# una-auxme/MeshGraphNets.jl

Measured on AMD Instinct MI355X. Metric: processor-step edges/s, higher is better.
Workload: dtype f32; 1 GPU; M-1M jittered-grid triangulation 1000x1000: N=1000000 nodes, E=5992002 directed edges, L=128, hidden_layers=2, 15 processor steps per bench step, fp32 storage, fp16x2 split MFMA (every fp32 operand = two fp16 pieces after a power-of-two scaling per weight chunk / per activation row, three exact piece products per fp32 product on v_mfma_f32_32x32x16_f16), fp32 accumulate; held to the fp32 tolerance; partition=single partition, edge_order=engine re-sorts by receiver once per trajectory (mgn_set_graph)

## Files before the change

### meshgraphnets.jl_amd/csrc/frag.hpp

```cpp
#pragma once
#include <hip/hip_runtime.h>
#include <stdint.h>

#include "kernels.h"

namespace mgn {

typedef float f32x16 __attribute__((ext_vector_type(16)));
typedef float f32x4 __attribute__((ext_vector_type(4)));
typedef float f32x2 __attribute__((ext_vector_type(2)));

#define DEVINL __device__ __forceinline__
#define PHASE_FENCE() __builtin_amdgcn_sched_barrier(0)
#define MGN_PRIO 1
#define OPAQUE_LANE()                          \
    int lane = lane0;                          \
    asm volatile("" : "+v"(lane));             \
    const int c = lane & 31, h = lane >> 5
constexpr float LN_EPS = 1e-5f;
constexpr int NUM_XCD = 8;

constexpr int STRIDE_ROW = 2, STRIDE_TILE = 64;

DEVINL const f32x4* row_ptr(const float* base, int64_t row, int L, int h) {
// ... 262 lines not shown
    const float rstd = ln_rstd(q * invL, gamma, 32 * NT);
    const f32x4* g4 = reinterpret_cast<const f32x4*>(gamma) + h;
    const f32x4* b4 = reinterpret_cast<const f32x4*>(beta) + h;
#pragma unroll
    for (int t = 0; t < NT; ++t)
#pragma unroll
        for (int g = 0; g < 4; ++g) {
            const f32x4 gv = g4[2 * (4 * t + g)];
            const f32x4 bv = b4[2 * (4 * t + g)];
#pragma unroll
            for (int i = 0; i < 4; ++i) x[t][4 * g + i] = x[t][4 * g + i] * rstd * gv[i] + bv[i];
        }
}

DEVINL void copy_to_lds(float* dst, const float* __restrict__ src, int nfloats) {
    const f32x4* s4 = reinterpret_cast<const f32x4*>(src);
    f32x4* d4 = reinterpret_cast<f32x4*>(dst);
    for (int i = threadIdx.x; i < nfloats / 4; i += blockDim.x) d4[i] = s4[i];
}

DEVINL void copy_to_lds_vec(f32x4* d4, const f32x4* __restrict__ s4, int n4) {
    constexpr int B = 8;
    const int bd = blockDim.x;
    for (int i = threadIdx.x; i < n4; i += B * bd) {
        f32x4 v[B];
#pragma unroll
        for (int u = 0; u < B; ++u) {
            const int k = i + u * bd;
            v[u] = s4[k < n4 ? k : i];
        }
#pragma unroll
        for (int u = 0; u < B; ++u) {
            const int k = i + u * bd;
            if (k < n4) d4[k] = v[u];
        }
    }
}

DEVINL void copy_to_lds_sel(float* dst, const float* __restrict__ src, int nfloats, bool fast) {
    if (fast) copy_to_lds_vec(reinterpret_cast<f32x4*>(dst), reinterpret_cast<const f32x4*>(src), nfloats / 4);
    else copy_to_lds(dst, src, nfloats);
}

#define MGN_COOP_PF 4
constexpr int COOP_PF = MGN_COOP_PF;

struct CoopRing {
    f32x4 r[COOP_PF];
};
DEVINL void coop_prime(CoopRing& ring, const float* wt, int lane) {
    const f32x4* wv = reinterpret_cast<const f32x4*>(wt) + lane;
#pragma unroll
    for (int p = 0; p < COOP_PF; ++p) ring.r[p] = wv[p * 64];
}
template <bool FENCE>
DEVINL void coop_chain_primed(f32x16& acc, const f32x16 (&in)[4], const float* wt, int lane, CoopRing& ring) {
    const f32x4* wv = reinterpret_cast<const f32x4*>(wt) + lane;
#pragma unroll
    for (int m = 0; m < 16; ++m) {
        const f32x4 a = ring.r[m % COOP_PF];
        if (m + COOP_PF < 16) ring.r[m % COOP_PF] = wv[(m + COOP_PF) * 64];
        if constexpr (FENCE) __builtin_amdgcn_sched_barrier(0);
#pragma unroll
        for (int i = 0; i < 4; ++i)
            acc = __builtin_amdgcn_mfma_f32_32x32x2f32(a[i], in[m >> 2][4 * (m & 3) + i], acc, 0, 0, 0);
        if constexpr (FENCE) __builtin_amdgcn_sched_barrier(0);
    }
}
template <bool FENCE>
DEVINL void coop_chain(f32x16& acc, const f32x16 (&in)[4], const float* wt, int lane) {
    CoopRing ring;
    coop_prime(ring, wt, lane);
    if constexpr (FENCE) __builtin_amdgcn_sched_barrier(0);
    coop_chain_primed<FENCE>(acc, in, wt, lane, ring);
}

DEVINL void coop_exchange(f32x16 (&full)[4], const f32x16& mine, f32x4* xch, int wave, int lane) {
#pragma unroll
    for (int g = 0; g < 4; ++g) {
        f32x4 v;
        v[0] = mine[4 * g + 0]; v[1] = mine[4 * g + 1]; v[2] = mine[4 * g + 2]; v[3] = mine[4 * g + 3];
        xch[(4 * wave + g) * 64 + lane] = v;
    }
    __syncthreads();
#pragma unroll
    for (int m = 0; m < 16; ++m) {
        const f32x4 v = xch[m * 64 + lane];
        full[m >> 2][4 * (m & 3) + 0] = v[0]; full[m >> 2][4 * (m & 3) + 1] = v[1];
        full[m >> 2][4 * (m & 3) + 2] = v[2]; full[m >> 2][4 * (m & 3) + 3] = v[3];
    }
}

DEVINL void tab_quarter(f32x16& q, const float* tab, int t, int h) { load_quarter(q, reinterpret_cast<const f32x4*>(tab) + h, 2, t); }

DEVINL void relu_quarter(f32x16& q) {
#pragma unroll
    for (int k = 0; k < 16; ++k) q[k] = fmaxf(q[k], 0.f);
}

DEVINL void zero_quarter(f32x16& q) {
#pragma unroll
    for (int k = 0; k < 16; ++k) q[k] = 0.f;
}

DEVINL void coop_layer_norm(f32x16& mine, const f32x16 (&full)[4], const float* gamma, const float* beta, int t, int h) {
    float s = 0.f;
#pragma unroll
    for (int u = 0; u < 4; ++u)
#pragma unroll
        for (int k = 0; k < 16; ++k) s += full[u][k];
    s += __shfl_xor(s, 32, 64);
    const float mean = s * (1.0f / 128);
    float q = 0.f;
#pragma unroll
    for (int u = 0; u < 4; ++u)
#pragma unroll
        for (int k = 0; k < 16; ++k) {
            const float d = full[u][k] - mean;
            q += d * d;
        }
    q += __shfl_xor(q, 32, 64);
    const float rstd = ln_rstd(q * (1.0f / 128), gamma, 128);
    f32x16 gq, bq;
    tab_quarter(gq, gamma, t, h);
    tab_quarter(bq, beta, t, h);
#pragma unroll
    for (int k = 0; k < 16; ++k) mine[k] = (mine[k] - mean) * rstd * gq[k] + bq[k];
}

DEVINL void coop_layer_norm_reg(f32x16& mine, const f32x16 (&full)[4], const f32x16& gq, const f32x16& bq, const float* lnp) {
    float s = 0.f;
#pragma unroll
    for (int u = 0; u < 4; ++u)
#pragma unroll
        for (int k = 0; k < 16; ++k) s += full[u][k];
    s += __shfl_xor(s, 32, 64);
    const float mean = s * (1.0f / 128);
    float q = 0.f;
#pragma unroll
    for (int u = 0; u < 4; ++u)
#pragma unroll
        for (int k = 0; k < 16; ++k) {
            const float d = full[u][k] - mean;
            q += d * d;
        }
    q += __shfl_xor(q, 32, 64);
    const float rstd = ln_rstd_at(q * (1.0f / 128), lnp);
#pragma unroll
    for (int k = 0; k < 16; ++k) mine[k] = (mine[k] - mean) * rstd * gq[k] + bq[k];
}

#define MGN_SPREAD_ROUNDS 24
#define MGN_SPREAD_ROUNDS_NODE MGN_SPREAD_ROUNDS
struct TileWalk {
    int tile, end, stride;
    DEVINL TileWalk(int ntiles, int wave, int spread_rounds = MGN_SPREAD_ROUNDS) {
        const int wpb = blockDim.x >> 6;
        const int xcd = blockIdx.x % NUM_XCD;
        const int per = (ntiles + NUM_XCD - 1) / NUM_XCD;
        const int nb = (gridDim.x - xcd + NUM_XCD - 1) / NUM_XCD;
        end = min(xcd * per + per, ntiles);
        stride = nb * wpb;
        const bool spread = per < spread_rounds * stride;
        tile = xcd * per + (spread ? wave * nb + (int)(blockIdx.x / NUM_XCD) : (int)(blockIdx.x / NUM_XCD) * wpb + wave);
    }
};


}
```

### meshgraphnets.jl_amd/csrc/split.hip

```cpp

#include "kernels.h"
#include "tile_common.hpp"
#include "split_common.hpp"
#include "launch.hpp"

namespace mgn {


template <int D> struct SpRing { u32x4 r2[D], r3[D]; };
template <bool G2, bool G3, bool RELU, int D, bool G1 = false, int OFF = 0, bool PRIMED = false, bool NEXT = false>
DEVINL void sp_layer_otf(f32x16 (&acc)[4], const f32x16 (&in)[4], const u32x4* p1, const u32x4* p2, const u32x4* p3, int lane,
                         SpRing<D>* carry = nullptr, const u32x4* nx2 = nullptr, const u32x4* nx3 = nullptr) {
    const u32x4* w1 = p1 + lane;
    const u32x4* w2 = p2 + lane;
    const u32x4* w3 = p3 + lane;
    const N16Buf b1 = n16_buf(G1 ? p1 : nullptr), b2 = n16_buf(G2 ? p2 : nullptr), b3 = n16_buf(G3 ? p3 : nullptr);
    const unsigned voff = (unsigned)lane * 16u;
#define SP_G1(IDX) n16_ldu(b1, voff, (IDX) * 1024)
#define SP_G2(IDX) n16_ldu(b2, voff, (IDX) * 1024)
#define SP_G3(IDX) n16_ldu(b3, voff, (IDX) * 1024)
    static_assert(!(PRIMED || NEXT) || !G1, "ring carry-over is written for the mid / lo streams");
    u32x4 r1[G1 ? D : 1], r2[G2 ? D : 1], r3[G3 ? D : 1];
    if constexpr (PRIMED) {
#pragma unroll
// ... 369 lines not shown
        EST(3);
        const int reff = ix.r >= 0 ? r : (-4 - c);
        const int rprev = lane_prev(reff);
        const int rnext = lane_next(reff);
        const bool head = (c == 0) || (reff != rprev);
        const unsigned hm = (unsigned)__ballot(head);
        const int start = 31 - __clz((int)(hm & (0xFFFFFFFFu >> (31 - c))));
        const int st_in = max(start, c & 16);
        const bool c1 = (c - 1 >= st_in), c2 = (c - 2 >= st_in), c4 = (c - 4 >= st_in), c8 = (c - 8 >= st_in);
        const bool cx = (c >= 16) && (start <= 15);
        EST(4);
        PHASE_FENCE();
        asm volatile("s_nop 1");
        RG_SCAN_LEVEL(acc, c1, "row_shr:1 row_mask:0xf bank_mask:0xf");
        RG_SCAN_LEVEL(acc, c2, "row_shr:2 row_mask:0xf bank_mask:0xf");
        RG_SCAN_LEVEL(acc, c4, "row_shr:4 row_mask:0xf bank_mask:0xf");
        RG_SCAN_LEVEL(acc, c8, "row_shr:8 row_mask:0xf bank_mask:0xf");
        RG_SCAN_LEVEL(acc, cx, "row_bcast:15 row_mask:0xa bank_mask:0xf");
        PHASE_FENCE();
        EST(5);
        const bool tail = valid && ((c == 31) || (reff != rnext));
        const int r_first = __builtin_amdgcn_readfirstlane(reff);
        const bool sl = (start == 0) && (ix.r_before == r_first);
        const bool sr = (c == 31) && (ix.r_after == reff);
        const bool to_carry = sl || sr;
        f32x4* dst = to_carry ? prow_ptr(a.CARRY, (int64_t)2 * tile + (sl ? 0 : 1), L, h) : tile_ptr(a.AGG, r >> 5, L, 32 * h + (r & 31));
        if (tail) store_frag<NT>(dst, to_carry ? STRIDE_PROW : STRIDE_TILE, acc);
        EST(6);
        PHASE_FENCE();
        load_frag<NT>(acc, prow_ptr(a.Q, ixn.r >= 0 ? ixn.r : 0, L, h), STRIDE_PROW);
        EST(7);
        ix = ixn;
        tw.tile += tw.stride;
    }
}

#define MGN_RINGH_AHEAD 2
template <int W>
struct Rh {
    static constexpr int WPL = 32 / W;
    static constexpr int NW = 3 * WPL;
    static constexpr int NB = MGN_RINGH_AHEAD + 1;
    static constexpr int BUF = W * 64;
    static_assert(NW % NB == 0 && NW % 2 == 0, "static window -> buffer / slot mapping");
};
template <int LPT> struct RhPend { u32x4 v[2][LPT]; };
struct RhFrag {
    u32x4 h, l;
};
template <int W, int LYR>
DEVINL RhFrag rh_first(const u32x4* hi, const u32x4* ring, int lane) {
    constexpr int b = (Rh<W>::WPL * LYR) % Rh<W>::NB;
    RhFrag f;
    f.h = hi[lane];
    f.l = ring[b * Rh<W>::BUF];
    return f;
}
struct RhSrc {
    const u32x4* lo[3];
};
template <int W, int LYR, int FIN, int RFS = 0, int NWV = 8, bool WRAP = false>
DEVINL void h2_layer_ring(f32x16 (&acc)[4], f32x16 (&in)[4], const u32x4* hi, const u32x4* hi_next, u32x4* ring, const RhSrc& src,
                          RhFrag& nx, RhPend<W / NWV>& pend, int lane, int tid, float sx, float cfin = 0.f, const float* btab = nullptr,
                          const f32x4* rf = nullptr, const N16Buf* rfb = nullptr) {
    constexpr int ROT = 2;
    constexpr int WPL = Rh<W>::WPL, NW = Rh<W>::NW, BUF = Rh<W>::BUF, NB = Rh<W>::NB, AHEAD = MGN_RINGH_AHEAD;
    f32x4 side[2 * ROT];
    if constexpr (!WRAP && RFS > 0) {
#pragma unroll
        for (int m = 0; m < 2 * ROT; ++m) side[m] = rf[m * RFS];
    }
    auto bias = [&](int sn, int u) {
        f32x2 b = {0.f, 0.f};
        if constexpr (FIN == 2) b = *reinterpret_cast<const f32x2*>(btab + 8 * (4 * (sn >> 1) + 2 * (sn & 1) + (u >> 1)) + 2 * (u & 1));
        return b;
    };
    unsigned ph[4], pl[4];
#pragma unroll
    for (int u = 0; u < 4; ++u) {
        const f32x2 b = bias(0, u);
        h2_split_pair<FIN>(ph[u], pl[u], in[0][2 * u], in[0][2 * u + 1], sx, cfin, b[0], b[1]);
    }
    constexpr int LPT = W / NWV;
    unsigned voff = (unsigned)tid * 16u;
    asm volatile("" : "+v"(voff));
    __builtin_amdgcn_sched_barrier(0);
#pragma unroll
    for (int s = 0; s < 8; ++s) {
        unsigned nh[4], nl[4];
#pragma unroll
        for (int t = 0; t < 4; ++t) {
            const int it = 4 * s + t;
            const int gw = WPL * LYR + it / W;
            const u32x4 a1 = nx.h, a2 = nx.l;
            if (it % W == 0) {
                const int g2 = (gw + AHEAD) % NW, l2 = g2 / WPL, w2 = g2 % WPL;
#pragma unroll
                for (int i = 0; i < LPT; ++i)
                    pend.v[AHEAD == 2 ? 0 : gw % 2][i] = *reinterpret_cast<const u32x4*>(reinterpret_cast<const char*>(src.lo[l2] + w2 * W * 64 + i * NWV * 64) + voff);
            }
            if constexpr (RFS > 0) {
                if ((t & 1) && s < 8 - ROT) {
                    f32x4 v;
                    if constexpr (WRAP) v = n16_ld(*rfb, (unsigned)lane * 16u, (2 * s + (t >> 1)) * 1024);
                    else v = rf[(2 * (s + ROT) + (t >> 1)) * RFS];
#pragma unroll
                    for (int i = 0; i < 4; ++i) in[s >> 1][8 * (s & 1) + 4 * (t >> 1) + i] = v[i];
                }
            }
            if (it + 1 < 32) {
                const int gn = WPL * LYR + (it + 1) / W;
                nx.h = hi[(it + 1) * 64 + lane];
                nx.l = ring[(gn % NB) * BUF + ((it + 1) % W) * 64];
            } else if (LYR < 2) {
                nx = rh_first<W, (LYR + 1) % 3>(hi_next, ring, lane);
            }
            if (it % W == W - 2) {
                const int b2 = (gw + 2) % NB;
                const int slot = AHEAD == 2 ? 0 : (gw + 1) % 2;
#pragma unroll
                for (int i = 0; i < LPT; ++i) ring[b2 * BUF + i * NWV * 64 + tid - lane] = pend.v[slot][i];
            }
            if (s < 7) {
                const int sn = s + 1;
                const f32x2 b = bias(sn, t);
                h2_split_pair<FIN>(nh[t], nl[t], in[sn >> 1][8 * (sn & 1) + 2 * t], in[sn >> 1][8 * (sn & 1) + 2 * t + 1], sx, cfin, b[0], b[1]);
            }
            const sp_f16x8 bh = h2_op(ph), bl = h2_op(pl);
            acc[t] = __builtin_amdgcn_mfma_f32_32x32x16_f16(h2_wop(a2), bh, acc[t], 0, 0, 0);
            acc[t] = __builtin_amdgcn_mfma_f32_32x32x16_f16(h2_wop(a1), bl, acc[t], 0, 0, 0);
            acc[t] = __builtin_amdgcn_mfma_f32_32x32x16_f16(h2_wop(a1), bh, acc[t], 0, 0, 0);
            __builtin_amdgcn_sched_barrier(0);
            if (it % W == W - 1) ring_barrier();
        }
#pragma unroll
        for (int u = 0; u < 4; ++u) {
            ph[u] = nh[u];
            pl[u] = nl[u];
        }
    }
    if constexpr (RFS > 0 && !WRAP) {
        f32x16 r[4];
#pragma unroll
        for (int u = 0; u < 8; ++u)
#pragma unroll
            for (int j = 0; j < 8; ++j)
                r[u >> 1][8 * (u & 1) + j] = u < ROT ? side[2 * u + (j >> 2)][j & 3] : in[(u - ROT) >> 1][8 * ((u - ROT) & 1) + j];
#pragma unroll
        for (int t = 0; t < 4; ++t) in[t] = r[t];
    }
}

#define MGN_RINGH_PHASE_UNITS 6
#define MGN_RINGH_W 8
template <int NWV>
__global__ __launch_bounds__(NWV * 64, NWV / 4) void k_edge_ring_h(const EdgeArgs a) {
    constexpr int NT = 4, L = 128, PC = 16384;
    constexpr int W = MGN_RINGH_W;
    constexpr int BUF = Rh<W>::BUF;
    extern __shared__ __attribute__((aligned(16))) float smem[];
    uint16_t* wl = reinterpret_cast<uint16_t*>(smem);
    copy_to_lds16(wl, a.splith[2], PC, true);
    copy_to_lds16(wl + PC, a.splith[0], PC, true);
    copy_to_lds16(wl + 2 * PC, a.splith[1], PC, true);
    const int lane0 = threadIdx.x & 63;
    const int wave = __builtin_amdgcn_readfirstlane(threadIdx.x >> 6);
    const int tid = (int)threadIdx.x;
    u32x4* ringbase = reinterpret_cast<u32x4*>(wl + 3 * PC);
    float* tb = reinterpret_cast<float*>(ringbase + Rh<W>::NB * BUF);
    copy_to_lds(tb, a.tabs, T_COUNT * L);
    RhSrc src;
    RhPend<W / NWV> pend;
    {
        const u32x4* g[3] = {reinterpret_cast<const u32x4*>(a.splith[2]), reinterpret_cast<const u32x4*>(a.splith[0]),
                             reinterpret_cast<const u32x4*>(a.splith[1])};
#pragma unroll
        for (int l = 0; l < 3; ++l) src.lo[l] = g[l] + 2048;
#pragma unroll
        for (int w = 0; w < 2; ++w)
#pragma unroll
            for (int i = 0; i < W / NWV; ++i) ringbase[w * BUF + i * NWV * 64 + tid] = src.lo[0][w * W * 64 + i * NWV * 64 + tid];
#pragma unroll
        for (int i = 0; i < W / NWV; ++i) {
            pend.v[1][i] = src.lo[(2 * W) / 32][((2 * W) % 32) * 64 + i * NWV * 64 + tid];
            pend.v[0][i] = pend.v[1][i];
        }
    }
    __syncthreads();
    const u32x4* l1h = reinterpret_cast<const u32x4*>(wl);
    const u32x4* l2h = reinterpret_cast<const u32x4*>(wl + PC);
    const u32x4* l3h = reinterpret_cast<const u32x4*>(wl + 2 * PC);
    const float sw1 = a.h2_s[2], rsw1 = a.h2_rs[2], rsw2 = a.h2_rs[0], rsw3 = a.h2_rs[1], b2pos = a.h2_b2pos;
    TileWalk tw0(a.ntiles, 0), tw(a.ntiles, wave);
    if (tw0.tile >= tw0.end) return;
    const int iters = (tw0.end - tw0.tile + tw0.stride - 1) / tw0.stride;
    if (MGN_RING_PHASES > 1 && iters >= 32) {
        const int ph = (int)(blockIdx.x / NUM_XCD) % MGN_RING_PHASES;
        for (int i = 0; i < ph * MGN_RINGH_PHASE_UNITS; ++i) __builtin_amdgcn_s_sleep(64);
    }
    const int last = a.tile0 + tw0.tile + (iters - 1) * tw0.stride;
    tw.tile += a.tile0;
    tw.end += a.tile0;
    auto clamp = [&](int t) { return t < tw.end ? t : last; };
    f32x16 acc[NT], y[NT];
    EdgeIdx ix = load_edge_idx_nb(a.snd, a.rcv, a.E, clamp(tw.tile), lane0 & 31);
    {
        const int h0 = lane0 >> 5;
        load_frag<NT>(acc, prow_ptr(a.Q, ix.r >= 0 ? ix.r : 0, L, h0), STRIDE_PROW);
        load_frag<NT>(y, tile_ptr(a.Elat, clamp(tw.tile), L, lane0), STRIDE_TILE);
    }
    int stamp_tile = 0;
    (void)stamp_tile;
    for (int j = 0; j < iters; ++j, ++stamp_tile) {
        OPAQUE_LANE();
        const bool on = tw.tile < tw.end;
        const int tile = clamp(tw.tile);
        const int nxt = clamp(tw.tile + tw.stride);
        const EdgeIdx ixn = load_edge_idx_nb(a.snd, a.rcv, a.E, nxt, c);
        const bool valid = on && ix.r >= 0;
        const int r = ix.r >= 0 ? ix.r : 0;
        f32x4* etile = tile_ptr(a.Elat, tile, L, lane);
        u32x4* ring = ringbase + lane;
        STAMP(0);
        __builtin_amdgcn_s_setprio(0);
        RhFrag nx = rh_first<W, 0>(l1h, ring, lane);
        const H2Scale x1 = h2_scale(h2_rowmax<true>(y));
        {
            const float cinv = x1.s * sw1;
#pragma unroll
            for (int t = 0; t < NT; ++t)
#pragma unroll
                for (int k = 0; k < 16; ++k) acc[t][k] *= cinv;
        }
        h2_layer_ring<W, 0, 0, STRIDE_PROW, NWV>(acc, y, l1h, l2h, ring, src, nx, pend, lane, tid, x1.s, 0.f, nullptr, prow_ptr(a.P, ix.s, L, h));
        {
            const float c1 = x1.rs * rsw1;
#pragma unroll
            for (int t = 0; t < NT; ++t)
#pragma unroll
                for (int k = 0; k < 16; ++k) acc[t][k] = __builtin_fmaf(acc[t][k], c1, y[t][k]);
        }
        CST(1);
        const H2Scale x2 = h2_scale(h2_rowmax<false>(acc));
        zero_frag<NT>(y);
        CST(2);
        h2_layer_ring<W, 1, 1, 0, NWV>(y, acc, l2h, l3h, ring, src, nx, pend, lane, tid, x2.s);
        CST(3);
        const float c2 = x2.rs * rsw2;
        const H2Scale x3 = h2_scale(__builtin_fmaf(h2_rowmax<false, true>(y), c2, b2pos));
        zero_frag<NT>(acc);
        CST(4);
        const f32x4* enext = tile_ptr(a.Elat, nxt, L, lane);
        const N16Buf enb = n16_buf(a.Elat + (int64_t)nxt * (TILE * L), TILE * L * 4);
        h2_layer_ring<W, 2, 2, STRIDE_TILE, NWV, true>(acc, y, l3h, l1h, ring, src, nx, pend, lane, tid, x3.s, c2, tb + T_B2 * L + 4 * h, enext, &enb);
        CST(5);
        EST(1);
        PHASE_FENCE();
        __builtin_amdgcn_s_setprio(MGN_PRIO);
        f32x16 er[NT];
        ring_load_e(er, etile);
#pragma unroll
        for (int m = 12; m < 16; ++m) {
            const f32x4 v = n16_ld(enb, (unsigned)lane * 16u, m * 1024);
#pragma unroll
            for (int i = 0; i < 4; ++i) y[3][4 * (m & 3) + i] = v[i];
        }
        {
            constexpr float invL = 1.0f / 128;
            const float c3 = x3.rs * rsw3;
            const f32x4* b34 = reinterpret_cast<const f32x4*>(tb + T_B3 * L) + h;
            float sm = 0.f;
#pragma unroll
            for (int t = 0; t < NT; ++t)
#pragma unroll
                for (int g = 0; g < 4; ++g) {
                    const f32x4 bv = b34[2 * (4 * t + g)];
#pragma unroll
                    for (int i = 0; i < 4; ++i) {
                        const float v = __builtin_fmaf(acc[t][4 * g + i], c3, bv[i]);
                        acc[t][4 * g + i] = v;
                        sm += v;
                    }
                }
            sm = half_sum(sm);
            const float mean = sm * invL;
            float q = 0.f;
#pragma unroll
            for (int t = 0; t < NT; ++t)
#pragma unroll
                for (int k = 0; k < 16; ++k) {
                    const float d = acc[t][k] - mean;
                    acc[t][k] = d;
                    q += d * d;
                }
            q = half_sum(q);
            const float rstd = ln_rstd_at(q * invL, tb + T_LN * L);
            const f32x4* g4 = reinterpret_cast<const f32x4*>(tb + T_GAMMA * L) + h;
            const f32x4* b4 = reinterpret_cast<const f32x4*>(tb + T_BETA * L) + h;
#pragma unroll
            for (int t = 0; t < NT; ++t) {
#pragma unroll
                for (int g = 0; g < 4; ++g) {
                    const f32x4 gv = g4[2 * (4 * t + g)];
                    const f32x4 bv = b4[2 * (4 * t + g)];
#pragma unroll
                    for (int i = 0; i < 4; ++i) acc[t][4 * g + i] = acc[t][4 * g + i] * rstd * gv[i] + bv[i];
// ... 476 lines not shown
    const u32x4* lqm = reinterpret_cast<const u32x4*>(wl + 3 * PC);
    const u32x4* gp = reinterpret_cast<const u32x4*>(a.split[4]);
    const u32x4* gq = reinterpret_cast<const u32x4*>(a.split[5]);
    const int lane0 = threadIdx.x & 63;
    const int wave = __builtin_amdgcn_readfirstlane(threadIdx.x >> 6);
    TileWalk tw(a.ntiles, wave, MGN_SPREAD_ROUNDS_NODE);
    if (tw.tile >= tw.end) return;
    f32x16 x[NT], acc[NT];
    load_frag<NT>(x, tile_ptr(a.V, a.tile0 + tw.tile, L, lane0), STRIDE_TILE);
    for (;;) {
        OPAQUE_LANE();
        const int tile = a.tile0 + tw.tile;
        const int next = tw.tile + tw.stride;
        const bool has_next = next < tw.end;
        const int n = tile * TILE + c;
        const bool valid = n < a.n;
        const int nn = valid ? n : 0;
        __builtin_amdgcn_s_setprio(0);
        zero_frag<NT>(acc);
        SpRing<D1> rg;
        sp_layer_otf<false, true, false, D1, false, 0, false, true>(acc, x, lph, lpm, gp + 4096, lane, &rg, nullptr, gq + 4096);
        __builtin_amdgcn_s_setprio(MGN_NODE_MPRIO);
        if (valid) store_frag<NT>(prow_ptr(a.P, nn, L, h), STRIDE_PROW, acc);
        __builtin_amdgcn_s_setprio(0);
        tab_frag<NT>(acc, tb + T_BQ * L, h);
        sp_layer_otf<false, true, false, D1, false, 32 % D1, true, false>(acc, x, lqh, lqm, gq + 4096, lane, &rg);
        __builtin_amdgcn_s_setprio(MGN_NODE_MPRIO);
        if (valid) store_frag<NT>(prow_ptr(a.Q, nn, L, h), STRIDE_PROW, acc);
        if (!has_next) break;
        PHASE_FENCE();
        load_frag<NT>(x, tile_ptr(a.V, a.tile0 + next, L, lane), STRIDE_TILE);
        tw.tile = next;
    }
}

#define MGN_SPH_D 8
#define MGN_NODE_VREFILL 6
__global__ __launch_bounds__(512, 2) void k_node_split_h(const NodeArgs a) {
    constexpr int NT = 4, L = 128, PC = 16384, D = MGN_SPH_D;
    static_assert(32 % D == 0, "the carried ring keeps offset 0 from chain to chain");
    extern __shared__ __attribute__((aligned(16))) float smem[];
    uint16_t* wl = reinterpret_cast<uint16_t*>(smem);
    {
        const bool fast = a.ntiles <= MGN_FAST_PRELOAD_TILES;
        copy_to_lds16(wl, a.splith[2], PC, fast);
        copy_to_lds16(wl + PC, a.splith[3], PC, fast);
        copy_to_lds16(wl + 2 * PC, a.splith[0], PC, fast);
        copy_to_lds16(wl + 3 * PC, a.splith[1], PC, fast);
    }
    float* tb = smem + 4 * PC / 2;
    copy_to_lds(tb, a.tabs, T_COUNT * L);
    __syncthreads();
    const u32x4* lvh = reinterpret_cast<const u32x4*>(wl);
    const u32x4* lah = reinterpret_cast<const u32x4*>(wl + PC);
    const u32x4* l2h = reinterpret_cast<const u32x4*>(wl + 2 * PC);
    const u32x4* l3h = reinterpret_cast<const u32x4*>(wl + 3 * PC);
    const u32x4* gv = reinterpret_cast<const u32x4*>(a.splith[2]) + 2048;
    const u32x4* ga = reinterpret_cast<const u32x4*>(a.splith[3]) + 2048;
    const u32x4* g2 = reinterpret_cast<const u32x4*>(a.splith[0]) + 2048;
    const u32x4* g3 = reinterpret_cast<const u32x4*>(a.splith[1]) + 2048;
    const float rswv = a.h2_rs[2], swa = a.h2_s[3], rswa = a.h2_rs[3], rsw2 = a.h2_rs[0], rsw3 = a.h2_rs[1], b2pos = a.h2_b2pos;
    const int lane0 = threadIdx.x & 63;
    const int wave = __builtin_amdgcn_readfirstlane(threadIdx.x >> 6);
    stagger_second_half(wave, a.stagger);
    TileWalk tw(a.ntiles, wave, MGN_SPREAD_ROUNDS_NODE);
    if (tw.tile >= tw.end) return;
    f32x16 x[NT], acc[NT];
    load_frag<NT>(x, tile_ptr(a.V, tw.tile, L, lane0), STRIDE_TILE);
    int stamp_tile = 0;
    (void)stamp_tile;
    for (;; ++stamp_tile) {
        OPAQUE_LANE();
        STAMP(0);
        const int tile = tw.tile;
        const int next = tile + tw.stride;
        const bool has_next = next < tw.end;
        const int n = tile * TILE + c;
        const bool valid = n < a.n;
        const int nn = valid ? n : 0;
        f32x4* vtile = tile_ptr(a.V, tile, L, lane);
        __builtin_amdgcn_s_setprio(0);
        SpRingH<D> rg;
        const H2Scale sv = h2_scale(h2_rowmax<true>(x));
        zero_frag<NT>(acc);
        h2_layer_otf<true, 0, D, 0, false, true>(acc, x, lvh, gv, lane, sv.s, 0.f, nullptr, &rg, ga);
        STAMP(1);
        LOAD_AGGREGATE(NT, x, a.rowptr, a.AGG, a.CARRY, a.zero_row);
        h2_finish_frag<NT>(acc, sv.rs * rswv, tb + T_B1 * L, h);
        const H2Scale sa = h2_scale(h2_rowmax<true>(x));
        h2_scale_frag<NT>(acc, sa.s * swa);
        STAMP(2);
        h2_layer_otf<true, 0, D, 0, true, true>(acc, x, lah, ga, lane, sa.s, 0.f, nullptr, &rg, g2);
        STAMP(3);
        const H2Scale s2 = h2_scale(h2_rowmax<false, true>(acc));
        zero_frag<NT>(x);
        h2_layer_otf<true, 1, D, 0, true, true>(x, acc, l2h, g2, lane, s2.s, 0.f, nullptr, &rg, g3);
        STAMP(4);
        const float c2 = s2.rs * rsw2 * (sa.rs * rswa);
        const H2Scale s3 = h2_scale(__builtin_fmaf(h2_rowmax<false, true>(x), c2, b2pos));
        zero_frag<NT>(acc);
        h2_layer_otf<true, 2, D, 0, true, false, MGN_NODE_VREFILL, STRIDE_TILE>(acc, x, l3h, g3, lane, s3.s, c2, tb + T_B2 * L + 4 * h, &rg, nullptr, vtile);
        STAMP(5);
        PHASE_FENCE();
        __builtin_amdgcn_s_setprio(MGN_NODE_MPRIO);
        h2_load_tail<MGN_NODE_VREFILL, STRIDE_TILE>(x, vtile);
        h2_finish_frag<NT>(acc, s3.rs * rsw3, tb + T_B3 * L, h);
        layer_norm_frag<NT>(acc, tb + T_GAMMA * L, tb + T_BETA * L, h);
#pragma unroll
        for (int t = 0; t < NT; ++t) x[t] += acc[t];
        STAMP(6);
        if (valid) store_frag<NT>(vtile, STRIDE_TILE, x);
        STAMP(7);
        if (!has_next) break;
        PHASE_FENCE();
        load_frag<NT>(x, tile_ptr(a.V, next, L, lane), STRIDE_TILE);
        tw.tile = next;
    }
}

__global__ __launch_bounds__(512, 2) void k_node_ring_hs(const NodeArgs a) {
    constexpr int NT = 4, L = 128, NWV = 8, NCH = 6;
    typedef RsT<NCH> R6;
    constexpr int BUF = Rs::BUF, LPT = BUF / (NWV * 64);
    extern __shared__ __attribute__((aligned(16))) float smem[];
    const int lane0 = threadIdx.x & 63;
    const int wave = __builtin_amdgcn_readfirstlane(threadIdx.x >> 6);
    const int tid = (int)threadIdx.x;
    u32x4* ringbase = reinterpret_cast<u32x4*>(smem);
    f32x4* park = reinterpret_cast<f32x4*>(ringbase + Rs::NB * BUF) + wave * 1024;
    float* tb = reinterpret_cast<float*>(ringbase + Rs::NB * BUF) + NWV * 4096;
    copy_to_lds(tb, a.tabs, T_COUNT * L);
    RsSrcT<NCH> src;
    u32x4 pend[Rs::SLOTS][LPT];
    {
        const int order[NCH] = {2, 3, 0, 1, 4, 5};
#pragma unroll
        for (int i = 0; i < NCH; ++i) src.w[i] = reinterpret_cast<const u32x4*>(a.splith[order[i]]);
#pragma unroll
        for (int w = 0; w < 2; ++w)
#pragma unroll
            for (int i = 0; i < LPT; ++i) ringbase[w * BUF + i * NWV * 64 + tid] = *rs_src(src.w[0], w, i * NWV * 64 + tid);
#pragma unroll
        for (int sl = 0; sl < Rs::SLOTS; ++sl)
#pragma unroll
            for (int i = 0; i < LPT; ++i) pend[sl][i] = *rs_src(src.w[0], 2, i * NWV * 64 + tid);
#pragma unroll
        for (int x = 2; x < Rs::AHEAD; ++x)
#pragma unroll
            for (int i = 0; i < LPT; ++i) pend[(x - Rs::AHEAD + R6::NW) % Rs::SLOTS][i] = *rs_src(src.w[x / Rs::WPL], x % Rs::WPL, i * NWV * 64 + tid);
    }
    __syncthreads();
    const float rswv = a.h2_rs[2], swa = a.h2_s[3], rswa = a.h2_rs[3], rsw2 = a.h2_rs[0], rsw3 = a.h2_rs[1], b2pos = a.h2_b2pos;
    const float rswp = a.h2_rs[4], rswq = a.h2_rs[5];
    TileWalk tw0(a.ntiles, 0, MGN_SPREAD_ROUNDS_NODE), tw(a.ntiles, wave, MGN_SPREAD_ROUNDS_NODE);
    if (tw0.tile >= tw0.end) return;
    const int iters = (tw0.end - tw0.tile + tw0.stride - 1) / tw0.stride;
    const int last = tw0.tile + (iters - 1) * tw0.stride;
    auto clamp = [&](int t) { return t < tw.end ? t : last; };
    f32x16 x[NT], acc[NT];
    load_frag<NT>(x, tile_ptr(a.V, clamp(tw.tile), L, lane0), STRIDE_TILE);
    int ra0, ra1;
    {
        const int n0 = clamp(tw.tile) * TILE + (lane0 & 31);
        ra0 = n0 < a.n ? a.rowptr[n0] : 0;
        ra1 = n0 < a.n ? a.rowptr[n0 + 1] : 0;
    }
    for (int j = 0; j < iters; ++j) {
        OPAQUE_LANE();
        const bool on = tw.tile < tw.end;
        const int tile = clamp(tw.tile);
        const int nxt = clamp(tw.tile + tw.stride);
        const int n = tile * TILE + c;
        const bool valid = on && n < a.n;
        const int nn = (n < a.n) ? n : 0;
        u32x4* ring = ringbase + lane;
        __builtin_amdgcn_s_setprio(0);
        RhFrag nx = rs_first<0>(ring);
#pragma unroll
        for (int m = 0; m < 16; ++m) {
            f32x4 v;
#pragma unroll
            for (int i = 0; i < 4; ++i) v[i] = x[m >> 2][4 * (m & 3) + i];
            park[m * 64 + lane] = v;
        }
        const H2Scale sv = h2_scale(h2_rowmax<true>(x));
        zero_frag<NT>(acc);
        hs_layer_ring<0, 0, 0, NWV, false, NCH>(acc, x, ring, src, nx, pend, lane, tid, sv.s);
        {
            const bool valid_row = n < a.n;
            const bool valid = valid_row;
            LOAD_AGGREGATE(NT, x, a.rowptr, a.AGG, a.CARRY, a.zero_row);
        }
        h2_finish_frag<NT>(acc, sv.rs * rswv, tb + T_B1 * L, h);
        const H2Scale sa = h2_scale(h2_rowmax<true>(x));
        h2_scale_frag<NT>(acc, sa.s * swa);
        hs_layer_ring<1, 0, 0, NWV, false, NCH>(acc, x, ring, src, nx, pend, lane, tid, sa.s);
        const H2Scale s2 = h2_scale(h2_rowmax<false, true>(acc));
        zero_frag<NT>(x);
        hs_layer_ring<2, 1, 0, NWV, false, NCH>(x, acc, ring, src, nx, pend, lane, tid, s2.s);
        const float c2 = s2.rs * rsw2 * (sa.rs * rswa);
        const H2Scale s3 = h2_scale(__builtin_fmaf(h2_rowmax<false, true>(x), c2, b2pos));
        zero_frag<NT>(acc);
        hs_layer_ring<3, 2, 0, NWV, false, NCH>(acc, x, ring, src, nx, pend, lane, tid, s3.s, c2, tb + T_B2 * L + 4 * h);
        PHASE_FENCE();
        __builtin_amdgcn_s_setprio(MGN_NODE_MPRIO);
        h2_finish_frag<NT>(acc, s3.rs * rsw3, tb + T_B3 * L, h);
        layer_norm_frag<NT>(acc, tb + T_GAMMA * L, tb + T_BETA * L, h);
#pragma unroll
        for (int m = 0; m < 16; ++m) {
            const f32x4 v = park[m * 64 + lane];
#pragma unroll
            for (int i = 0; i < 4; ++i) x[m >> 2][4 * (m & 3) + i] = v[i] + acc[m >> 2][4 * (m & 3) + i];
        }
        if (valid) store_frag<NT>(tile_ptr(a.V, tile, L, lane), STRIDE_TILE, x);
        PHASE_FENCE();
        __builtin_amdgcn_s_setprio(0);
        const H2Scale sp = h2_scale(h2_rowmax<true>(x));
        zero_frag<NT>(acc);
        hs_layer_ring<4, 0, 0, NWV, false, NCH>(acc, x, ring, src, nx, pend, lane, tid, sp.s);
        __builtin_amdgcn_s_setprio(MGN_NODE_MPRIO);
        h2_scale_frag<NT>(acc, sp.rs * rswp);
        if (valid) store_frag<NT>(prow_ptr(a.P, nn, L, h), STRIDE_PROW, acc);
        __builtin_amdgcn_s_setprio(0);
        zero_frag<NT>(acc);
        const N16Buf vnb = n16_buf(a.V + (int64_t)nxt * (TILE * L), TILE * L * 4);
        hs_layer_ring<5, 0, STRIDE_TILE, NWV, true, NCH>(acc, x, ring, src, nx, pend, lane, tid, sp.s, 0.f, nullptr, nullptr, &vnb);
        __builtin_amdgcn_s_setprio(MGN_NODE_MPRIO);
#pragma unroll
        for (int m = 12; m < 16; ++m) {
            const f32x4 v = n16_ld(vnb, (unsigned)lane * 16u, m * 1024);
#pragma unroll
            for (int i = 0; i < 4; ++i) x[3][4 * (m & 3) + i] = v[i];
        }
        {
            const int n1 = nxt * TILE + c;
            ra0 = n1 < a.n ? a.rowptr[n1] : 0;
            ra1 = n1 < a.n ? a.rowptr[n1 + 1] : 0;
        }
        h2_finish_frag<NT>(acc, sp.rs * rswq, tb + T_BQ * L, h);
        if (valid) store_frag<NT>(prow_ptr(a.Q, nn, L, h), STRIDE_PROW, acc);
        tw.tile += tw.stride;
    }
}

__global__ __launch_bounds__(512, 2) void k_project_split_h(const NodeArgs a) {
    constexpr int NT = 4, L = 128, PC = 16384;
    extern __shared__ __attribute__((aligned(16))) float smem[];
    uint16_t* wl = reinterpret_cast<uint16_t*>(smem);
    {
        const bool fast = a.ntiles <= MGN_FAST_PRELOAD_TILES;
        copy_to_lds16(wl, a.splith[4], 2 * PC, fast);
        copy_to_lds16(wl + 2 * PC, a.splith[5], 2 * PC, fast);
    }
    float* tb = smem + 4 * PC / 2;
    copy_to_lds(tb, a.tabs, T_COUNT * L);
    __syncthreads();
    const u32x4* lph = reinterpret_cast<const u32x4*>(wl);
    const u32x4* lpl = reinterpret_cast<const u32x4*>(wl + PC);
    const u32x4* lqh = reinterpret_cast<const u32x4*>(wl + 2 * PC);
    const u32x4* lql = reinterpret_cast<const u32x4*>(wl + 3 * PC);
    const float rswp = a.h2_rs[4], rswq = a.h2_rs[5];
    const int lane0 = threadIdx.x & 63;
    const int wave = __builtin_amdgcn_readfirstlane(threadIdx.x >> 6);
    TileWalk tw(a.ntiles, wave, MGN_SPREAD_ROUNDS_NODE);
    if (tw.tile >= tw.end) return;
    f32x16 x[NT], acc[NT];
    load_frag<NT>(x, tile_ptr(a.V, a.tile0 + tw.tile, L, lane0), STRIDE_TILE);
    for (;;) {
        OPAQUE_LANE();
        const int tile = a.tile0 + tw.tile;
        const int next = tw.tile + tw.stride;
        const bool has_next = next < tw.end;
        const int n = tile * TILE + c;
        const bool valid = n < a.n;
        const int nn = valid ? n : 0;
        __builtin_amdgcn_s_setprio(0);
        const H2Scale sv = h2_scale(h2_rowmax<true>(x));
        zero_frag<NT>(acc);
        h2_layer_otf<false, 0, 1>(acc, x, lph, lpl, lane, sv.s);
        __builtin_amdgcn_s_setprio(MGN_NODE_MPRIO);
        h2_scale_frag<NT>(acc, sv.rs * rswp);
        if (valid) store_frag<NT>(prow_ptr(a.P, nn, L, h), STRIDE_PROW, acc);
        __builtin_amdgcn_s_setprio(0);
        zero_frag<NT>(acc);
        h2_layer_otf<false, 0, 1>(acc, x, lqh, lql, lane, sv.s);
        __builtin_amdgcn_s_setprio(MGN_NODE_MPRIO);
        h2_finish_frag<NT>(acc, sv.rs * rswq, tb + T_BQ * L, h);
        if (valid) store_frag<NT>(prow_ptr(a.Q, nn, L, h), STRIDE_PROW, acc);
        if (!has_next) break;
        PHASE_FENCE();
        load_frag<NT>(x, tile_ptr(a.V, a.tile0 + next, L, lane), STRIDE_TILE);
        tw.tile = next;
    }
}

hipError_t launch_edge_ring(const EdgeArgs& a, const LaunchCfg& lc, hipStream_t s) {
    if (lc.threads == 256) return launch_kernel(k_edge_ring<4>, lc.blocks, lc.threads, lc.lds, s, a);
    return launch_kernel(k_edge_ring<8>, lc.blocks, lc.threads, lc.lds, s, a);
}
static Switch g_ringh_stream{"MGN_RINGH_STREAM", 1};
int edge_ring_h_streamed() { return g_ringh_stream; }
int set_ringh_stream(int on) { return g_ringh_stream.set(on); }
hipError_t launch_edge_ring_h(const EdgeArgs& a, const LaunchCfg& lc, hipStream_t s) {
    if (g_ringh_stream) {
        LaunchCfg ls = lc;
        ls.lds = (size_t)Rs::NB * Rs::BUF * 16 + (size_t)(lc.threads / 64) * 16384 + (size_t)T_COUNT * 128 * 4 + 64;
        if (lc.threads == 256) return launch_kernel(k_edge_ring_hs<4>, ls.blocks, ls.threads, ls.lds, s, a);
        return launch_kernel(k_edge_ring_hs<8>, ls.blocks, ls.threads, ls.lds, s, a);
    }
// ... 67 lines not shown
```

Before: 1.990 billion edges/s.

## Phase node-kernel tile walk into staggered block groups with start delays

Replaces the node kernel's per-XCD tile walk with a phased walk that divides blocks into groups and reorders tile positions so the remainder round falls on specific blocks. Blocks that get one round fewer are assigned a late-start group and sleep before beginning, which staggers their memory and compute phases against the other groups. The aim is to reduce contention at kernel start and balance the tail. The cost is idle sleep cycles and more complex index math, and an untuned sleep length could delay completion.

```diff
diff --git a/meshgraphnets.jl_amd/csrc/frag.hpp b/meshgraphnets.jl_amd/csrc/frag.hpp
--- a/meshgraphnets.jl_amd/csrc/frag.hpp
+++ b/meshgraphnets.jl_amd/csrc/frag.hpp
@@ -438,17 +438,46 @@
 
 #define MGN_SPREAD_ROUNDS 24
 #define MGN_SPREAD_ROUNDS_NODE MGN_SPREAD_ROUNDS
+struct WalkPos {
+    int tile, stride, end, rounds, late;
+};
+#define MGN_HD __host__ __device__ __forceinline__
+MGN_HD constexpr WalkPos tile_walk(int ntiles, int grid, int wpb, int block, int wave, int spread_rounds) {
+    const int xcd = block % NUM_XCD, blk = block / NUM_XCD;
+    const int per = (ntiles + NUM_XCD - 1) / NUM_XCD;
+    const int nb = (grid - xcd + NUM_XCD - 1) / NUM_XCD;
+    const int end = xcd * per + per < ntiles ? xcd * per + per : ntiles;
+    const int stride = nb * wpb;
+    const bool spread = per < spread_rounds * stride;
+    const int first0 = xcd * per + (spread ? blk : blk * wpb);
+    const int rounds = first0 < end ? (end - first0 + stride - 1) / stride : 0;
+    return WalkPos{xcd * per + (spread ? wave * nb + blk : blk * wpb + wave), stride, end, rounds, 0};
+}
+MGN_HD constexpr WalkPos phased_walk(int ntiles, int grid, int wpb, int block, int wave, int G, int spread_rounds, int min_rounds) {
+    const WalkPos w = tile_walk(ntiles, grid, wpb, block, wave, spread_rounds);
+    const int xcd = block % NUM_XCD, blk = block / NUM_XCD;
+    const int nb = w.stride / wpb;
+    const int start = xcd * ((ntiles + NUM_XCD - 1) / NUM_XCD);
+    const int t = w.end - start;
+    if (G <= 1 || t <= 0) return w;
+    const int full = t / w.stride, rem = t % w.stride;
+    if (rem == 0 || full < min_rounds) return w;
+    const int g = blk % G, idx = blk / G;
+    const int nbg = (nb - g + G - 1) / G;
+    const int before = g * (nb / G) + (g < nb % G ? g : nb % G);
+    const bool spread = (ntiles + NUM_XCD - 1) / NUM_XCD < spread_rounds * w.stride;
+    const int pos0 = before * wpb + (spread ? idx : idx * wpb);
+    const int pos = before * wpb + (spread ? wave * nbg + idx : idx * wpb + wave);
+    const int rounds = full + (pos0 < rem ? 1 : 0);
+    return WalkPos{start + pos, w.stride, w.end, rounds, rounds == full ? g : 0};
+}
 struct TileWalk {
     int tile, end, stride;
     DEVINL TileWalk(int ntiles, int wave, int spread_rounds = MGN_SPREAD_ROUNDS) {
-        const int wpb = blockDim.x >> 6;
-        const int xcd = blockIdx.x % NUM_XCD;
-        const int per = (ntiles + NUM_XCD - 1) / NUM_XCD;
-        const int nb = (gridDim.x - xcd + NUM_XCD - 1) / NUM_XCD;
-        end = min(xcd * per + per, ntiles);
-        stride = nb * wpb;
-        const bool spread = per < spread_rounds * stride;
-        tile = xcd * per + (spread ? wave * nb + (int)(blockIdx.x / NUM_XCD) : (int)(blockIdx.x / NUM_XCD) * wpb + wave);
+        const WalkPos w = tile_walk(ntiles, (int)gridDim.x, (int)(blockDim.x >> 6), (int)blockIdx.x, wave, spread_rounds);
+        tile = w.tile;
+        end = w.end;
+        stride = w.stride;
     }
 };
 
diff --git a/meshgraphnets.jl_amd/csrc/split.hip b/meshgraphnets.jl_amd/csrc/split.hip
--- a/meshgraphnets.jl_amd/csrc/split.hip
+++ b/meshgraphnets.jl_amd/csrc/split.hip
@@ -545,6 +545,15 @@
 }
 
 #define MGN_RINGH_PHASE_UNITS 6
+#ifndef MGN_NODE_PHASES
+#define MGN_NODE_PHASES 2
+#endif
+#ifndef MGN_NODE_PHASE_UNITS
+#define MGN_NODE_PHASE_UNITS 22
+#endif
+#ifndef MGN_NODE_PHASE_MIN_ROUNDS
+#define MGN_NODE_PHASE_MIN_ROUNDS 1
+#endif
 #define MGN_RINGH_W 8
 template <int NWV>
 __global__ __launch_bounds__(NWV * 64, NWV / 4) void k_edge_ring_h(const EdgeArgs a) {
@@ -1327,9 +1336,11 @@
     __syncthreads();
     const float rswv = a.h2_rs[2], swa = a.h2_s[3], rswa = a.h2_rs[3], rsw2 = a.h2_rs[0], rsw3 = a.h2_rs[1], b2pos = a.h2_b2pos;
     const float rswp = a.h2_rs[4], rswq = a.h2_rs[5];
-    TileWalk tw0(a.ntiles, 0, MGN_SPREAD_ROUNDS_NODE), tw(a.ntiles, wave, MGN_SPREAD_ROUNDS_NODE);
-    if (tw0.tile >= tw0.end) return;
-    const int iters = (tw0.end - tw0.tile + tw0.stride - 1) / tw0.stride;
+    const WalkPos tw0 = phased_walk(a.ntiles, (int)gridDim.x, NWV, (int)blockIdx.x, 0, MGN_NODE_PHASES, MGN_SPREAD_ROUNDS_NODE, MGN_NODE_PHASE_MIN_ROUNDS);
+    WalkPos tw = phased_walk(a.ntiles, (int)gridDim.x, NWV, (int)blockIdx.x, wave, MGN_NODE_PHASES, MGN_SPREAD_ROUNDS_NODE, MGN_NODE_PHASE_MIN_ROUNDS);
+    const int iters = tw0.rounds;
+    if (iters <= 0) return;
+    for (int i = 0; i < tw0.late * MGN_NODE_PHASE_UNITS / MGN_NODE_PHASES; ++i) __builtin_amdgcn_s_sleep(64);
     const int last = tw0.tile + (iters - 1) * tw0.stride;
     auto clamp = [&](int t) { return t < tw.end ? t : last; };
     f32x16 x[NT], acc[NT];
```

Result: no change. 2.003 billion edges/s, median of 6 (+0.7%).
